# pymc-devs/pymc

Measured on AMD Instinct MI355X. Metric: effective samples/sec (and leapfrog steps/sec), 10k-param hierarchical logistic regression, one NUTS chain per GPU, higher is better.
Workload: dtype f64

## Files before the change

### pymc_amd/csrc/engine.hip

```cpp
#include <hip/hip_runtime.h>

#include <algorithm>
#include <atomic>
#include <chrono>
#include <cmath>
#include <cstdio>
#include <cstdlib>
#include <cstring>
#include <mutex>
#include <thread>
#include <utility>
#include <ctime>
#include <string>
#include <vector>

#include "kernels.h"
#include "small_kernel.h"
#include "mixture_kernel.h"
#include "nuts_mi355.h"
#include "pcg64_stream.h"
#include "advi.h"

static thread_local std::string g_err;

// ... 1135 lines not shown
      const auto& uses = cs.lin_uses[l][k];
      if (uses.size() > LIN_MAXUSE) { g_err = "a linear predictor column is read by too many factors (LIN_MAXUSE)"; return false; }
      C.n_use = (int32_t)uses.size();
      for (size_t u = 0; u < uses.size(); ++u) { C.adj_off[u] = uses[u].adj_off; C.use_size[u] = uses[u].size; }
      const int64_t last = (int64_t)L.off[k] + (int64_t)(L.P - 1) * L.stride[k];
      if (L.off[k] < 0 || L.stride[k] < 0 || (L.stride[k] == 0 && L.P > 1)) { g_err = "linear predictor: bad coefficient offset / stride"; return false; }
      double* dst_base = nullptr; int64_t cbase = 0;
      if (L.var[k] >= 0) {
        if (L.var[k] >= md.n_vars) { g_err = "linear predictor refers to a missing variable"; return false; }
        const VarDev& v = cs.vars[L.var[k]];
        if (last >= v.size) { g_err = "linear predictor: coefficients beyond the end of their variable"; return false; }
        C.transform = v.transform; C.lower = v.lower; C.upper = v.upper;
        cbase = v.offset; dst_base = md.lin_gdense + v.offset;
      } else {
        const int fi = -(L.var[k] + 1);
        int t = -1;
        for (int u = 0; u < md.n_derived; ++u) if (md.derived_f[u] == fi) t = u;
        if (t < 0) { g_err = "linear predictor: coefficients must be a variable or a NUTS_D_DERIVED factor"; return false; }
        const int64_t sz = cs.fac[fi].size;
        if (last >= sz) { g_err = "linear predictor: coefficients beyond the end of their derived vector"; return false; }
        C.transform = -1; C.lower = 0.0; C.upper = 0.0;
        cbase = md.derived_off[t]; dst_base = const_cast<double*>(md.pool) + md.derived_off[t] + sz;
      }
      for (int p = 0; p < L.P; ++p) {
        const int64_t e = (int64_t)L.off[k] + (int64_t)p * L.stride[k];
        coef[(size_t)k * L.P + p] = (int32_t)(cbase + e);
        if (C.n_use > 0) srcs.push_back(Src{(int64_t)reinterpret_cast<intptr_t>(dst_base + e), LinSrc{l, k, p, 0}, dst_base + e});
      }
    }
    D.coef = m->keep(dev_upload(coef.data(), coef.size()));
    m->alg_bytes += 16 * L.N * (int64_t)L.P;
  }
  std::stable_sort(srcs.begin(), srcs.end(), [](const Src& a, const Src& b) { return a.key < b.key; });
  std::vector<LinTarget> targets;
  std::vector<LinSrc> flat;
  for (size_t i = 0; i < srcs.size(); ++i) {
    if (i == 0 || srcs[i].key != srcs[i - 1].key) targets.push_back(LinTarget{srcs[i].dst, (int32_t)flat.size(), 0});
    targets.back().n_src++;
    flat.push_back(srcs[i].src);
  }
  md.n_lins = s->n_lins; md.n_lin_targets = (int32_t)targets.size();
  md.lins = m->keep(dev_upload(m->lins_host.data(), m->lins_host.size()));
  md.lin_targets = m->keep(dev_upload(targets.data(), targets.size()));
  md.lin_srcs = m->keep(dev_upload(flat.data(), flat.size()));
  return true;
}

static bool build_rows_group(nuts_model* m, const nuts_model_spec* s, const std::vector<int64_t>& gptr, const std::vector<int32_t>& tile0,
                             int64_t maxT, int W, int gpw) {
  RowsDev& lg = m->md.lg;
  const int n = m->md.n, D = lg.D, SPAN = WAVE * m->rows_rpl;
  const int64_t n_tiles = tile0[lg.G];
  lg.ga = 1; lg.ga_w = gpw ? GB_W : W;
  lg.ga_gpw = gpw;
  lg.ga_bsz = gpw ? gpw : (lg.G + 31) / 32;
  lg.ga_flags = env_int("NUTS_GA_FLAGS", 0);
  lg.ga_T_uni = 0; lg.ga_ng_uni = 0;
  {
    bool uni = lg.G > 0;
    for (int g = 1; g < lg.G; ++g) uni = uni && (gptr[g + 1] - gptr[g] == gptr[1] - gptr[0]);
    if (uni && maxT > 0) { lg.ga_T_uni = (int32_t)maxT; lg.ga_ng_uni = gptr[1] - gptr[0]; }
  }
  lg.ga_nblk = (lg.G + lg.ga_bsz - 1) / lg.ga_bsz;
  lg.ga_auxel = n - lg.G * D;
  lg.ga_naux = m->ga_struct_ok == 2 ? (lg.ga_auxel + WAVE * lg.ga_w - 1) / (WAVE * lg.ga_w) : 0;
  lg.ga_nrec = lg.ga_nblk + lg.ga_naux;
  bool ones0 = D == 8 && env_int("NUTS_GA_ONES0", 1) != 0 && lg.N > 0;
  for (int64_t i = 0; ones0 && i < lg.N; ++i) ones0 = s->rows_X[i * D] == 1.0;
  const int DX = ones0 ? D - 1 : D;
  lg.ga_dx = DX;
  const int64_t TS = (int64_t)DX * SPAN, GA_SKEW = env_int("NUTS_GA_SKEW", DX == 7 || DX == 5 ? 1120 : 1056);
  if (GA_SKEW % DX != 0) return refuse("NUTS_GA_SKEW must be a multiple of the stored column count");
  std::vector<int64_t> coff((size_t)lg.G * W, 0);
  int64_t pos = 0, max_ct = 0;
  for (int g = 0; g < lg.G; ++g) {
    const int64_t T = tile0[g + 1] - tile0[g];
    for (int w = 0; w < W; ++w) {
      const int64_t ct = (int64_t)(w + 1) * T / W - (int64_t)w * T / W;
      coff[(size_t)g * W + w] = pos;
      pos += ct * TS + GA_SKEW;
      max_ct = std::max(max_ct, ct);
    }
  }
  lg.ga_cstride_uni = 0;
  if (lg.ga_T_uni > 0 && lg.ga_T_uni % W == 0) {
    lg.ga_cstride_uni = (lg.ga_T_uni / W) * TS + GA_SKEW;
  } else lg.ga_T_uni = 0;
  lg.Npad = n_tiles * SPAN; lg.n_spans = n_tiles;
  std::vector<double> xt((size_t)(pos + TS), 0.0);
  std::vector<int8_t> yy((size_t)(pos / DX + 2 * SPAN), 0);
  for (int g = 0; g < lg.G; ++g) {
    const int64_t T = tile0[g + 1] - tile0[g];
    for (int64_t i = gptr[g]; i < gptr[g + 1]; ++i) {
      const int64_t r = i - gptr[g], t = r / SPAN, rr = r % SPAN;
      int w = (int)(((t + 1) * W - 1) / std::max<int64_t>(T, 1));
      while (w > 0 && (int64_t)w * T / W > t) --w;
      while (w + 1 < W && (int64_t)(w + 1) * T / W <= t) ++w;
      const int64_t base = coff[(size_t)g * W + w] + (t - (int64_t)w * T / W) * TS;
      for (int d = D - DX; d < D; ++d) xt[(size_t)(base + (int64_t)(d - (D - DX)) * SPAN + rr)] = s->rows_X[i * D + d];
      yy[(size_t)(base / DX + rr)] = s->rows_y[i];
    }
  }
  lg.Xt = m->keep(dev_upload(xt.data(), xt.size()));
  lg.y = m->keep(dev_upload(yy.data(), yy.size()));
  m->rows_xt_len = (int64_t)xt.size(); m->rows_y_len = (int64_t)yy.size();
  lg.ga_coff = m->keep(dev_upload(coff.data(), coff.size()));
  lg.ga_tile0 = m->keep(dev_upload(tile0.data(), tile0.size()));
  lg.ga_part = m->keep(dev_alloc<double>((size_t)lg.G * PART_STRIDE));
  const size_t bpart_len = gpw ? 2 * (size_t)PART_STRIDE * ((lg.ga_nrec + WAVE - 1) / WAVE * WAVE) : 2 * (size_t)lg.ga_nrec * PART_STRIDE;
  lg.ga_bpart = m->keep(dev_alloc<double>(bpart_len));
  lg.ga_ticket = m->keep(dev_alloc<unsigned>(lg.ga_nblk));
  if (lg.ga_part) hipMemset(lg.ga_part, 0, (size_t)lg.G * PART_STRIDE * sizeof(double));
  if (lg.ga_bpart) hipMemset(lg.ga_bpart, 0, bpart_len * sizeof(double));
  if (lg.ga_ticket) hipMemset(lg.ga_ticket, 0, lg.ga_nblk * sizeof(unsigned));
  m->rows_grid = gpw ? lg.ga_nblk : lg.G;
  return true;
}

static bool build_rows_spans(nuts_model* m, const nuts_model_spec* s, int cus) {
  RowsDev& lg = m->md.lg;
  const int D = lg.D, SPAN = WAVE * m->rows_rpl;
  const int32_t* gid = s->rows_gid;
  int wpc = env_int("NUTS_ROWS_WAVES_PER_CU", 0);
  if (wpc <= 0) {
    const int64_t spans = (s->rows_N + (int64_t)WAVE * m->rows_rpl - 1) / ((int64_t)WAVE * m->rows_rpl);
    wpc = spans >= (int64_t)cus * 32 * 4 ? 32 : 16;
  }
  {
    std::vector<double> xt((size_t)D * lg.Npad, 0.0);
    for (int64_t i = 0; i < lg.N; ++i) {
      const int64_t sp = i / SPAN, r = i % SPAN;
      for (int d = 0; d < D; ++d) xt[((size_t)sp * D + d) * SPAN + r] = s->rows_X[i * D + d];
    }
    lg.Xt = m->keep(dev_upload(xt.data(), xt.size()));
  }
  std::vector<int8_t> yy(lg.Npad, 0);
  for (int64_t i = 0; i < lg.N; ++i) yy[i] = s->rows_y[i];
  lg.y = m->keep(dev_upload(yy.data(), yy.size()));
  const int waves_per_block = ROWS_BLOCK / WAVE;
  int64_t want_waves = std::min<int64_t>((int64_t)cus * wpc, lg.n_spans);
  const int nb_main = (int)((want_waves + waves_per_block - 1) / waves_per_block);
  lg.n_waves = nb_main * waves_per_block;
  std::vector<int32_t> span_gid(lg.n_spans), mixed_g0, mixed_seg_base, mixed_seg_gid;
  std::vector<int64_t> mixed_span;
  for (int64_t sp = 0; sp < lg.n_spans; ++sp) {
    const int64_t r0 = sp * SPAN, r1 = r0 + SPAN;
    if (r1 <= lg.N && gid[r0] == gid[r1 - 1]) { span_gid[sp] = gid[r0]; continue; }
    span_gid[sp] = -1;
    mixed_span.push_back(sp);
    mixed_g0.push_back(gid[r0]);
    mixed_seg_base.push_back((int32_t)mixed_seg_gid.size());
    int prev = -1;
    for (int64_t r = r0; r < std::min<int64_t>(r1, lg.N); ++r)
      if (gid[r] != prev) { prev = gid[r]; mixed_seg_gid.push_back(prev); }
  }
  lg.n_mixed = (int32_t)mixed_span.size();
  lg.n_mixed_seg = (int32_t)mixed_seg_gid.size();
  std::vector<int32_t> run_ptr(lg.n_waves + 1, 0), seg_gid;
  std::vector<int4> runs;
  for (int w = 0; w < lg.n_waves; ++w) {
    const int64_t s0 = (int64_t)w * lg.n_spans / lg.n_waves, s1 = (int64_t)(w + 1) * lg.n_spans / lg.n_waves;
    run_ptr[w] = (int32_t)runs.size();
    for (int64_t sp = s0; sp < s1; ++sp) {
      if (span_gid[sp] < 0) continue;
      if (!runs.empty() && (int)runs.size() > run_ptr[w] && runs.back().z == span_gid[sp] && runs.back().x + runs.back().y == sp) {
        runs.back().y++;
// ... 354 lines not shown
  if (hipGetDeviceCount(&ndev) != hipSuccess || ndev == 0) {
    g_err = "no HIP device visible: libnuts_mi355 requires an MI355X (gfx950); there is no CPU fallback";
    return nullptr;
  }
  auto* m = new nuts_model();
  if (!model_build(m, s)) { nuts_model_destroy(m); return nullptr; }
  return m;
}

extern "C" int nuts_model_set_data(nuts_model* m, int32_t data_id, const double* values, int64_t n) {
  if (!m || !values) { g_err = "null argument"; return NUTS_E_ARG; }
  if (data_id < 0 || data_id >= (int)m->data_refs.size()) { g_err = "nuts_model_set_data: no such data vector"; return NUTS_E_ARG; }
  const nuts_data_ref& r = m->data_refs[data_id];
  if (n != r.size) { g_err = "nuts_model_set_data: the length of a data vector cannot change"; return NUTS_E_ARG; }
  HIPCHK(hipStreamSynchronize(m->stream));
  HIPCHK(hipMemcpy(const_cast<double*>(m->md.pool) + r.offset, values, (size_t)n * sizeof(double), hipMemcpyHostToDevice));
  m->data_epoch++;
  return NUTS_OK;
}

extern "C" int nuts_model_set_data_many(nuts_model* m, int32_t count, const int32_t* data_ids, const double* values, const int64_t* lens) {
  if (!m || count < 0 || (count > 0 && (!data_ids || !values || !lens))) { g_err = "null argument"; return NUTS_E_ARG; }
  int64_t total = 0;
  for (int i = 0; i < count; ++i) {
    if (data_ids[i] < 0 || data_ids[i] >= (int)m->data_refs.size()) { g_err = "nuts_model_set_data_many: no such data vector"; return NUTS_E_ARG; }
    if (lens[i] != m->data_refs[data_ids[i]].size) { g_err = "nuts_model_set_data_many: the length of a data vector cannot change"; return NUTS_E_ARG; }
    total += lens[i];
  }
  if (total == 0) return NUTS_OK;
  if (m->set_pin_len < total) {
    if (m->set_ev) HIPCHK(hipEventSynchronize(m->set_ev));
    if (m->set_pin) hipHostFree(m->set_pin);
    m->set_pin = nullptr; m->set_pin_len = 0;
    HIPCHK(hipHostMalloc((void**)&m->set_pin, (size_t)total * sizeof(double), hipHostMallocDefault));
    m->set_pin_len = total;
  }
  if (!m->set_ev) HIPCHK(hipEventCreateWithFlags(&m->set_ev, hipEventDisableTiming));
  else HIPCHK(hipEventSynchronize(m->set_ev));
  std::memcpy(m->set_pin, values, (size_t)total * sizeof(double));
  int64_t at = 0;
  for (int i = 0; i < count;) {
    const int64_t off0 = m->data_refs[data_ids[i]].offset;
    int64_t run = lens[i];
    int j = i + 1;
    while (j < count && m->data_refs[data_ids[j]].offset == off0 + run) { run += lens[j]; ++j; }
    if (run > 0)
      HIPCHK(hipMemcpyAsync(const_cast<double*>(m->md.pool) + off0, m->set_pin + at, (size_t)run * sizeof(double), hipMemcpyHostToDevice, m->stream));
    at += run;
    i = j;
  }
  HIPCHK(hipEventRecord(m->set_ev, m->stream));
  m->data_epoch++;
  return NUTS_OK;
}

static void group_remove_model(struct nuts_group* g, nuts_model* m);
extern "C" void nuts_model_destroy(nuts_model* m) {
  if (!m) return;
  if (m->stream) hipStreamSynchronize(m->stream);
  if (m->set_ev) hipEventDestroy(m->set_ev);
  if (m->set_pin) hipHostFree(m->set_pin);
  if (m->group) group_remove_model(m->group, m);
  for (void* p : m->owned) if (p) hipFree(p);
  for (auto e : m->ev) hipEventDestroy(e);
  if (m->host_pin) hipHostFree(m->host_pin);
  if (m->own_stream) hipStreamDestroy(m->own_stream);
  delete m;
}

extern "C" int nuts_model_debug_ticks(nuts_model* m, int64_t* out) {
  if (!m || !out) return NUTS_E_ARG;
  HIPCHK(hipStreamSynchronize(m->stream));
  HIPCHK(hipMemcpy(out, m->md.ticks, 64 * sizeof(long long), hipMemcpyDeviceToHost));
  return NUTS_OK;
}

extern "C" int32_t nuts_model_ndim(const nuts_model* m) { return m ? m->md.n : -1; }
extern "C" int nuts_model_get_scalar(const nuts_model* m, const char* name, double* out) {
  if (!m || !name || !out) return NUTS_E_ARG;
  const std::string k(name);
  if (k == "rows_group_aligned") *out = m->md.lg.ga;
  else if (k == "rows_group_block") *out = m->md.lg.ga_gpw;
  else if (k == "rows_aux_workgroups") *out = m->md.lg.ga ? m->md.lg.ga_naux : 0;
  else if (k == "mixture_workgroups") *out = m->md.has_mix ? m->md.mix.nwg : 0;
  else if (k == "glm_workgroups") *out = m->md.has_glm ? m->md.glm.nwg : 0;
  else if (k == "glm_row_stride") *out = m->md.has_glm ? m->md.glm.xstride : 0;
  else if (k == "glm_layout_width") *out = m->md.has_glm ? m->md.glm.Ppad : 0;
  else if (k == "mvn_row_aligned") *out = m->md.has_mvn ? m->md.mv.aligned : 0;
  else if (k == "rows_waves") *out = m->md.lg.ga ? m->md.lg.ga_w : m->md.lg.n_waves;
  else if (k == "lean") *out = m->md.lean_ok;
  else if (k == "chain_group_kind") {
    const RowsDev& lg = m->md.lg;
    const bool is_mvn = m->md.has_mvn && (m->md.mv.aligned == 4 || m->md.mv.aligned == 8 || m->md.mv.aligned == 16);
    const bool is_rows = m->md.has_logit && !m->md.has_mvn && lg.ga && lg.ga_naux == 0 && lg.D == 8 && m->ga_struct_ok == 1;
    *out = is_mvn ? 1.0 : (is_rows ? (lg.ga_gpw > 0 ? 3.0 : 2.0) : 0.0);
  }
  else if (k == "chain_group_wide_ok") *out = (m->md.has_mvn && m->md.mv.aligned > 0 && m->md.mv.k % 16 == 0) ? 1.0 : 0.0;
  else if (k == "chain_group_wide_rows") *out = 8.0;
  else if (k == "single_workgroup_ok") *out = (m->md.n <= SMALL_MAX_N && m->ept == 1 && !m->md.has_logit && !m->md.has_mvn && !m->md.has_mix && !m->md.has_glm && m->md.n_lins == 0 && m->factor_elems <= SMALL_MAX_ELEMS) ? 1.0 : 0.0;
  else { g_err = "unknown model scalar " + k; return NUTS_E_ARG; }
  return NUTS_OK;
}
extern "C" int64_t nuts_model_algorithmic_bytes(const nuts_model* m) { return m ? m->alg_bytes : 0; }

extern "C" int nuts_model_logp_grad(nuts_model* m, const double* q, double* logp, double* grad) {
  if (!m || !q || !logp) { g_err = "null argument"; return NUTS_E_ARG; }
  const int n = m->md.n;
  std::memcpy(m->host_pin, q, n * sizeof(double));
  HIPCHK(hipMemcpyAsync(m->q_dev, m->host_pin, n * sizeof(double), hipMemcpyHostToDevice, m->stream));
  m->md.fdead_mode = 1;
  model_enqueue_plain(m, m->q_dev, m->g_dev, m->lp_dev);
  m->md.fdead_mode = 0;
  HIPCHK(hipMemcpyAsync(m->host_pin + n, m->g_dev, n * sizeof(double), hipMemcpyDeviceToHost, m->stream));
  HIPCHK(hipMemcpyAsync(m->host_pin + 2 * n, m->lp_dev, sizeof(double), hipMemcpyDeviceToHost, m->stream));
  HIPCHK(hipStreamSynchronize(m->stream));
  HIPCHK(hipGetLastError());
  *logp = m->host_pin[2 * n];
  if (m->md.n_factors > 0 && !std::isfinite(*logp)) {
    std::vector<int32_t> fd(m->md.n_factors);
    HIPCHK(hipMemcpy(fd.data(), m->md.fdead, fd.size() * sizeof(int32_t), hipMemcpyDeviceToHost));
    bool any = false;
    for (int32_t v : fd) any = any || v != 0;
    if (any) {
      if (grad) {
        m->md.fdead_mode = 2;
        model_enqueue_plain(m, m->q_dev, m->g_dev, m->lp_dev);
        m->md.fdead_mode = 0;
        HIPCHK(hipMemcpyAsync(m->host_pin + n, m->g_dev, n * sizeof(double), hipMemcpyDeviceToHost, m->stream));
      }
      HIPCHK(hipMemsetAsync(m->md.fdead, 0, fd.size() * sizeof(int32_t), m->stream));
      HIPCHK(hipStreamSynchronize(m->stream));
      HIPCHK(hipGetLastError());
    }
  }
  if (grad) std::memcpy(grad, m->host_pin + n, n * sizeof(double));
  return NUTS_OK;
}

static void profile_enable(nuts_model* m, bool on, int sample_every, size_t max_pairs) {
  m->profile = on;
  m->sample_every = std::max(1, sample_every);
  m->ev_used = 0;
  m->dom_launches = 0;
  m->dom_units = 0;
  m->run_open = 0; m->runs_seen = 0;
  while (on && m->ev.size() < 2 * max_pairs) {
    hipEvent_t e;
    hipEventCreate(&e);
    m->ev.push_back(e);
  }
  m->ev_units.assign(m->ev.size() / 2 + 1, 1);
}
static double profile_sum_ms(nuts_model* m, int64_t* pairs) {
  std::vector<float> ms(m->ev_used / 2, 0.f);
  std::vector<double> run_avg;
  for (size_t i = 0; i + 1 < m->ev_used; i += 2) {
    if (hipEventElapsedTime(&ms[i / 2], m->ev[i], m->ev[i + 1]) != hipSuccess) ms[i / 2] = -1.f;
    else if (m->ev_units[i / 2] > 1) run_avg.push_back(ms[i / 2] / m->ev_units[i / 2]);
  }
  double med = 0.0;
  if (!run_avg.empty()) { std::sort(run_avg.begin(), run_avg.end()); med = run_avg[run_avg.size() / 2]; }
  double tot = 0.0;
  int64_t units = 0, kept = 0;
  for (size_t p = 0; p < ms.size(); ++p) {
    if (ms[p] < 0.f) continue;
    const int u = m->ev_units[p];
// ... 2070 lines not shown
```

### pymc_amd/csrc/model_dev.h

```cpp
#pragma once
#include "device_math.h"
#include "nuts_mi355.h"

#define MAX_BTERMS 8
#define MAX_DERIVED 4
#define MAX_FACTOR_BT 6
#define MAX_DEFERRED 256
#define LOGIT_MAXD 8
#define SEG_MAIN_MAX 10

struct VarDev {
  int32_t offset, size, transform, deferred;
  double lower, upper;
  int32_t normal_prior;
  int32_t def_base;
  double np_mu, np_inv_var, np_lognorm;
};

struct Contrib {
  int32_t f;
  int16_t arg, slot;
  int32_t owner;
  int32_t fast;
  int32_t dist, pad;
  double konst;
  double p[4];
};

#define MAX_GSLOTS 64
struct GSlot { int32_t var, did; int64_t adj_off; };
struct GSweepFactor { int32_t f, slot0, n_slots, elem0; int32_t orphan, pad; };
#define GADJ_LONG 512
#define GADJ_CHUNK 4096
struct GLong { int64_t adj_off; int32_t lst_off, len; int32_t nchunk, pad; };

struct FactorBT {
  int32_t n, pad;
  struct { int16_t arg, slot; int32_t bterm; } e[MAX_FACTOR_BT];
};

struct RowsDev {
  int64_t N, Npad;
  int32_t D, G;
  const double* Xt;
  const int8_t* y;
  const int64_t* gptr;
  int32_t off_mu, off_sigma, off_z, sigma_tr;
  int32_t var_mu, var_sigma, var_z, pad;
  int32_t def_mu, def_sigma;
  int32_t segK, seg_pad;
  int64_t n_spans;
  int32_t n_waves, n_seg;
  const int32_t* run_ptr;
  const int4* runs;
  const int32_t* gseg_ptr;
  double* seg_part;
  int32_t n_mixed, n_mixed_seg;
  const int64_t* mixed_span;
  const int32_t* mixed_g0;
  const int32_t* mixed_seg_base;
  const int32_t* gmix_ptr;
  double* mixed_part;
  double* wave_lp;
  int32_t ga, ga_w;
  int32_t ga_dx, ga_gpw;
  int32_t ga_nblk, ga_bsz;
  int32_t ga_T_uni, ga_flags;
  int64_t ga_ng_uni;
  const int32_t* ga_tile0;
  const int64_t* ga_coff;
  int64_t ga_cstride_uni;
  unsigned* ga_ticket;
  double* ga_part;
  double* ga_bpart;
  int32_t ga_naux, ga_nrec, ga_auxel, ga_pad2;
  double z_np_mu, z_np_inv_var, z_np_lognorm;
  double mu_c[3];
  double sg_c[2];
};

struct MvnDev {
  int32_t k, off;
  const double* mu;
  const double* prec;
  double konst;
  double* rowq;
  double* gdense;
  const double* winv; const double* winv_t;
  double* wy;
  int32_t aligned, al_nwg;
  double* al_part;
};

#define MIX_MAXK 16
struct MixDev {
  int64_t N;
  int32_t K, off_mu, off_sigma, off_w;
  int32_t tr_sigma, nwg;
  int32_t w_simplex, pad_;
  double alpha[MIX_MAXK], w_konst;
  const double* y;
  const double* assign;
  double sigma_c[MIX_MAXK], logw_c[MIX_MAXK];
  double* part;
  double* gdense;
  double* lp;
};

struct GlmDev {
  int64_t N;
  int32_t P, Ppad;
  int32_t xstride, xpad_;
  int32_t family, lpr, ch;
  int32_t off_beta, off_icpt, off_sigma, tr_sigma, nwg;
  const double* beta_buf; double* beta_seed;
  double sigma_c;
  double konst;
  const double* X;
  const double* Xt;
  const double* y;
  double* part;
  double* gdense;
  double* lp;
};

#define SW_LEAF 6
#define SWL_DATA 0
#define SWL_GATHER 1
// ... 909 lines not shown
```

### pymc_amd/csrc/rows_ga_kernel.h

```cpp
#pragma once
#include "rows_kernel.h"

__device__ __forceinline__ void ga_def_local(const RowsDev& R, bool is_mu, double qn, double& gx, double& dxdq, double& dj, double& lp) {
  if (is_mu) {
    const double r = qn - R.mu_c[0];
    const double z = r * R.mu_c[1];
    lp = -0.5 * z * z - R.mu_c[2] + (-0.91893853320467274178);
    gx = -z * R.mu_c[1]; dxdq = 1.0; dj = 0.0;
  } else {
    double x, lj;
    if (R.sigma_tr == NUTS_TR_LOG) { x = exp(qn); dxdq = x; lj = qn; dj = 1.0; }
    else { x = qn; dxdq = 1.0; lj = 0.0; dj = 0.0; }
    const double z = x * R.sg_c[0];
    double lpf = -0.5 * z * z - R.sg_c[1] + (-0.22579135264472743236);
    double g = -z * R.sg_c[0];
    if (!(x >= 0)) { lpf = -INFINITY; g = 0.0; }
    gx = g; lp = lj + lpf;
  }
}

template <int D, int RPL>
__device__ __forceinline__ void ga_load(const RowsDev& R, int64_t xoff, int lane, double (&x)[D][RPL], uint32_t& ybits) {
  constexpr int SPAN = WAVE * RPL;
  const double* tile = R.Xt + xoff + lane * RPL;
  const int8_t* yp = R.y + xoff / D + lane * RPL;
  if (RPL == 2) ybits = *reinterpret_cast<const uint16_t*>(yp);
  else ybits = *reinterpret_cast<const uint32_t*>(yp);
#pragma unroll
  for (int d = 0; d < D; ++d) {
#pragma unroll
    for (int k = 0; k < RPL; k += 2) {
      const double2 a = *reinterpret_cast<const double2*>(tile + d * SPAN + k);
      x[d][k] = a.x; x[d][k + 1] = a.y;
    }
  }
}

typedef double ga_v2d __attribute__((ext_vector_type(2)));
struct GaTileRegs { ga_v2d c[8]; uint32_t y; };

__device__ __forceinline__ void ga_issue8(const double* base , const int8_t* ybase,
                                          uint32_t voff16, uint32_t voff2, GaTileRegs& t) {
  const double* base2 = base + 512;
  asm volatile(
      "s_nop 4\n\t"
      "global_load_dwordx4 %0, %9, %10\n\t"
      "global_load_dwordx4 %1, %9, %10 offset:1024\n\t"
      "global_load_dwordx4 %2, %9, %10 offset:2048\n\t"
      "global_load_dwordx4 %3, %9, %10 offset:3072\n\t"
      "global_load_dwordx4 %4, %9, %11\n\t"
      "global_load_dwordx4 %5, %9, %11 offset:1024\n\t"
      "global_load_dwordx4 %6, %9, %11 offset:2048\n\t"
      "global_load_dwordx4 %7, %9, %11 offset:3072\n\t"
      "global_load_ushort %8, %12, %13"
      : "=&v"(t.c[0]), "=&v"(t.c[1]), "=&v"(t.c[2]), "=&v"(t.c[3]), "=&v"(t.c[4]), "=&v"(t.c[5]), "=&v"(t.c[6]), "=&v"(t.c[7]), "=&v"(t.y)
      : "v"(voff16), "s"(base), "s"(base2), "v"(voff2), "s"(ybase)
      : "memory");
}

template <int N>
__device__ __forceinline__ void ga_wait8(GaTileRegs& t) {
  asm volatile("s_waitcnt vmcnt(%9)"
               : "+v"(t.c[0]), "+v"(t.c[1]), "+v"(t.c[2]), "+v"(t.c[3]), "+v"(t.c[4]), "+v"(t.c[5]), "+v"(t.c[6]), "+v"(t.c[7]), "+v"(t.y)
               : "i"(N));
}

struct GaTileRegs7 { ga_v2d c[7]; uint32_t y; };

__device__ __forceinline__ void ga_issue8(const double* base, const int8_t* ybase, uint32_t voff16, uint32_t voff2, GaTileRegs7& t) {
  const double* base2 = base + 512;
  asm volatile(
      "s_nop 4\n\t"
      "global_load_dwordx4 %0, %8, %9\n\t"
      "global_load_dwordx4 %1, %8, %9 offset:1024\n\t"
      "global_load_dwordx4 %2, %8, %9 offset:2048\n\t"
      "global_load_dwordx4 %3, %8, %9 offset:3072\n\t"
      "global_load_dwordx4 %4, %8, %10\n\t"
      "global_load_dwordx4 %5, %8, %10 offset:1024\n\t"
      "global_load_dwordx4 %6, %8, %10 offset:2048\n\t"
      "global_load_ushort %7, %11, %12"
      : "=&v"(t.c[0]), "=&v"(t.c[1]), "=&v"(t.c[2]), "=&v"(t.c[3]), "=&v"(t.c[4]), "=&v"(t.c[5]), "=&v"(t.c[6]), "=&v"(t.y)
      : "v"(voff16), "s"(base), "s"(base2), "v"(voff2), "s"(ybase)
      : "memory");
}

template <int N>
__device__ __forceinline__ void ga_wait8(GaTileRegs7& t) {
  asm volatile("s_waitcnt vmcnt(%8)"
               : "+v"(t.c[0]), "+v"(t.c[1]), "+v"(t.c[2]), "+v"(t.c[3]), "+v"(t.c[4]), "+v"(t.c[5]), "+v"(t.c[6]), "+v"(t.y)
               : "i"(N));
}

__device__ __forceinline__ void ga_unpack(const GaTileRegs& t, double (&xx)[8][2]) {
#pragma unroll
  for (int dd = 0; dd < 8; ++dd) { xx[dd][0] = t.c[dd].x; xx[dd][1] = t.c[dd].y; }
}
__device__ __forceinline__ void ga_unpack(const GaTileRegs7& t, double (&xx)[8][2]) {
  xx[0][0] = 1.0; xx[0][1] = 1.0;
#pragma unroll
  for (int dd = 1; dd < 8; ++dd) { xx[dd][0] = t.c[dd - 1].x; xx[dd][1] = t.c[dd - 1].y; }
}
template <int DX> struct GaTileSel { typedef GaTileRegs type; };
template <> struct GaTileSel<7> { typedef GaTileRegs7 type; };

template <int D, int RPL, bool ILV = false>
__device__ __forceinline__ void ga_tile(const double (&x)[D][RPL], uint32_t yb, const double (&beta)[D], int nvalid, int lane,
                                        double (&acc)[D], double& lp) {
  if constexpr (ILV && RPL == 2) {
    double eta[2] = {0.0, 0.0}, yk[2], l[2], rr[2];
#pragma unroll
    for (int d = 0; d < D; ++d) { eta[0] = fma(x[d][0], beta[d], eta[0]); eta[1] = fma(x[d][1], beta[d], eta[1]); }
    yk[0] = (double)(yb & 0xffu); yk[1] = (double)((yb >> 8) & 0xffu);
    logit_row2(eta, yk, l, rr);
#pragma unroll
    for (int k = 0; k < 2; ++k) {
      const bool in = lane * 2 + k < nvalid;
      lp += in ? l[k] : 0.0;
      rr[k] = in ? rr[k] : 0.0;
    }
#pragma unroll
    for (int d = 0; d < D; ++d) { acc[d] = fma(rr[0], x[d][0], acc[d]); acc[d] = fma(rr[1], x[d][1], acc[d]); }
    return;
  }
#pragma unroll
  for (int k = 0; k < RPL; ++k) {
    double eta = 0.0;
#pragma unroll
    for (int d = 0; d < D; ++d) eta = fma(x[d][k], beta[d], eta);
    double l, rr;
    logit_row(eta, (double)((yb >> (8 * k)) & 0xffu), l, rr);
    const bool in = lane * RPL + k < nvalid;
    lp += in ? l : 0.0;
    rr = in ? rr : 0.0;
#pragma unroll
    for (int d = 0; d < D; ++d) acc[d] = fma(rr, x[d][k], acc[d]);
    if constexpr (!ILV) __builtin_amdgcn_sched_barrier(0);
  }
}

#define GA_MAXW 4
#define GA_MAXCHUNK 8
#define GA_F_NOTAIL 1

struct GaArgs;
template <int D>
__device__ __forceinline__ void ga_tail(const GaArgs& T, int g, double (&s_acc)[4][2][D + 1], double (&s_red)[NDOT],
                                        double (&s_cp)[8][PART_STRIDE], int (&s_info)[4], double (&s_keep)[5][WAVE]);

struct GaArgs {
  ModelDev md; ArenaDev A; EvalIO io;
  int j, rev, fold, par, d, max_depth;
  double Emax;
  HostStatus* st;
  EvalIO cio;
  int cj, cd, cseq, cpad;
};
#define GA_FOLD_CTL 1
#define GA_FOLD_SRC 2
#include "rows_aux.h"

template <int D>
__device__ __forceinline__ void ga_hyper(const ModelDev& md, const QView& qv, int fold, int par, int lane, double& hval0, double& hph0) {
  const RowsDev& R = md.lg;
  if (fold & GA_FOLD_SRC) {
    const LeanSrc prev = lean_src(md, par ^ 1);
    rows_hyper_fold_elem<D>(R, prev.part, prev.stride, prev.nblk, prev.def_loc, qv, lane, hval0, hph0);
  } else {
    const int e = lane % (2 * D);
    const int i = e < D ? R.off_mu + e : R.off_sigma + (e - D);
    if (qv.composed) { hph0 = qv.p_half(i); hval0 = fma(qv.eps, qv.var[i] * hph0, qv.q[i]); }
    else { hph0 = 0.0; hval0 = qv.q[i]; }
  }
}

template <int D, int RPL, int DX = D>
__global__ __launch_bounds__(64 * GA_MAXW, 4) void k_rows_ga(GaArgs a) {
  constexpr int SPAN = WAVE * RPL;
  static_assert(DX == D || (D == 8 && DX == 7), "only the intercept column of an 8-column model is elided");
  typedef typename GaTileSel<DX>::type Tile;
  constexpr int LOADS = DX + 1;
  const ModelDev& md = a.md;
  const ArenaDev& A = a.A;
  const EvalIO& io = a.io;
  const int j = a.j, rev = a.rev, fold = a.fold, par = a.par, d = a.d, max_depth = a.max_depth;
  const double Emax = a.Emax;
  HostStatus* const st = a.st;
  const RowsDev& R = md.lg;
  int b = (int)blockIdx.x;
  if (fold & GA_FOLD_CTL) {
    if (b == 0) { control_lean(md, A, a.cio, a.cj, a.cd, Emax, max_depth, st, a.cseq, lean_src(md, par ^ 1)); return; }
    --b;
  }
  const int g = b;
  const int tid = threadIdx.x, lane = tid & (WAVE - 1), w = __builtin_amdgcn_readfirstlane(tid >> 6), W = (int)blockDim.x >> 6;
  Leaf lf; QView qv;
  const int aborted = load_aborted(io, A);
  resolve_leaf(io, A, j, lf, qv);
  const bool leaf = io.mode != MODE_PLAIN;
  __shared__ double s_acc[GA_MAXW][2][D + 1];
  __shared__ double s_red[NDOT];
  __shared__ double s_cp[GA_MAXCHUNK][PART_STRIDE];
  __shared__ int s_info[4];
  __shared__ double s_keep[5][WAVE];
  __shared__ __attribute__((aligned(16))) char s_args[(sizeof(GaArgs) + 15) / 16 * 16];
  __shared__ __attribute__((aligned(16))) char s_auxprog[GA_AUX_PROG_LDS];
  if (b >= R.G) {
    static_assert(GA_AUX_SCRATCH_DOUBLES(GA_MAXW) <= GA_MAXCHUNK * PART_STRIDE, "auxiliary scratch does not fit the chunk buffer");
    double hv, hp;
    ga_hyper<D>(md, qv, fold, par, lane, hv, hp);
    const int aux_id = b - R.G;
    ga_aux<4>((const GaArgs*)__builtin_amdgcn_kernarg_segment_ptr(), aux_id, hv, hp, &s_cp[0][0], GA_MAXW, s_auxprog,
                R.ga_bpart + ((int64_t)par * R.ga_nrec + R.ga_nblk + aux_id) * PART_STRIDE, 1);
    return;
  }

  int T; int64_t ng, cbase;
  if (R.ga_T_uni > 0) { T = R.ga_T_uni; ng = R.ga_ng_uni; cbase = (int64_t)(g * W + w) * R.ga_cstride_uni; }
  else {
    T = __builtin_amdgcn_readfirstlane(R.ga_tile0[g + 1] - R.ga_tile0[g]);
    ng = __builtin_amdgcn_readfirstlane((int)(R.gptr[g + 1] - R.gptr[g]));
    const int64_t cb = R.ga_coff[g * W + w];
    cbase = ((int64_t)__builtin_amdgcn_readfirstlane((int)(cb >> 32)) << 32) | (uint32_t)__builtin_amdgcn_readfirstlane((int)(cb & 0xffffffffll));
  }
  const int c0 = (int)((int64_t)w * T / W), c2 = (int)((int64_t)(w + 1) * T / W);
  const int n = c2 - c0;
  const int nA = (n + 1) / 2;
  const int nsw = rev ? n - nA : nA;
  constexpr int64_t TS = (int64_t)DX * SPAN;
  auto local_at = [&](int i) { return rev ? (i < nsw ? nA + i : i - nsw) : i; };
  auto tile_at = [&](int i) { return cbase + (int64_t)local_at(i) * TS; };
  const int l_last = (c2 == T) ? n - 1 : -1;
  const int n_last = (int)(ng - (int64_t)(T - 1) * SPAN);
  double xa[D][RPL], xb[D][RPL];
  uint32_t ya = 0, yb = 0;
  Tile ta, tb;
  if constexpr (D == 8 && RPL == 2) {
    const uint32_t voff16 = (uint32_t)lane * 16u, voff2 = (uint32_t)lane * 2u;
    const int64_t o0 = tile_at(0), o1 = tile_at(min(1, max(n - 1, 0)));
    ga_issue8(R.Xt + o0, R.y + o0 / DX, voff16, voff2, ta);
    ga_issue8(R.Xt + o1, R.y + o1 / DX, voff16, voff2, tb);
  } else {
    ga_load<D, RPL>(R, tile_at(0), lane, xa, ya);
  }
  if (lane == 0) {
#pragma unroll
    for (int dd = 0; dd <= D; ++dd) { s_acc[w][0][dd] = 0.0; s_acc[w][1][dd] = 0.0; }
  }
  {
    const uint4* ka = (const uint4*)__builtin_amdgcn_kernarg_segment_ptr();
    for (int t = tid; t < (int)((sizeof(GaArgs) + 15) / 16); t += (int)blockDim.x) reinterpret_cast<uint4*>(s_args)[t] = ka[t];
  }
  __syncthreads();

  double hval0, hph0;
  ga_hyper<D>(md, qv, fold, par, lane, hval0, hph0);
  const int dl = lane % D;
  const int iz = R.off_z + g * D + dl;
  double beta[D];
  {
    double zq, zph;
    if (qv.composed) { zph = fma(qv.half, qv.g[iz], qv.p[iz]); zq = fma(qv.eps, qv.var[iz] * zph, qv.q[iz]); }
    else { zph = 0.0; zq = qv.q[iz]; }
    const double m_lane = __shfl(hval0, dl);
    const double sraw = __shfl(hval0, D + dl);
    const double s_lane = R.sigma_tr == NUTS_TR_LOG ? exp(sraw) : sraw;
    const double bl = fma(s_lane, zq, m_lane);
#pragma unroll
    for (int dd = 0; dd < D; ++dd) beta[dd] = readlane_d(bl, dd);
    if (w == 0) { s_keep[0][lane] = hval0; s_keep[1][lane] = hph0; s_keep[2][lane] = zq; s_keep[3][lane] = zph; s_keep[4][lane] = s_lane; }
  }
  if (aborted) return;

  {
    double acc[D], lp = 0.0;
#pragma unroll
    for (int dd = 0; dd < D; ++dd) acc[dd] = 0.0;
    int half = rev ? 1 : 0;
    auto flush = [&]() {
#pragma unroll
      for (int dd = 0; dd < D; ++dd) {
        const double sum = wave_sum(acc[dd]);
        if (lane == 0) s_acc[w][half][dd] = sum;
        acc[dd] = 0.0;
      }
      const double sum = wave_sum(lp);
      if (lane == 0) s_acc[w][half][D] = sum;
      lp = 0.0;
      half ^= 1;
    };
#define GA_STAGE(X, Y, I)                                                                   \
    {                                                                                        \
      if ((I) == nsw) flush();                                                               \
      ga_tile<D, RPL>(X, Y, beta, local_at(I) == l_last ? n_last : SPAN, lane, acc, lp);     \
    }
    const int nm1 = n - 1;
    if constexpr (D == 8 && RPL == 2) {
      const uint32_t voff16 = (uint32_t)lane * 16u, voff2 = (uint32_t)lane * 2u;
      auto issue = [&](int i, Tile& t) {
        const int64_t off = tile_at(min(i, nm1));
        ga_issue8(R.Xt + off, R.y + off / DX, voff16, voff2, t);
      };
#define GA_ASTAGE(T, I)                                                                      \
      {                                                                                      \
        ga_wait8<LOADS>(T);                                                                  \
        if ((I) == nsw) flush();                                                             \
        double xx[8][2];                                                                     \
        ga_unpack(T, xx);                                                                    \
        ga_tile<8, 2>(xx, T.y, beta, local_at(I) == l_last ? n_last : SPAN, lane, acc, lp); \
      }
      for (int i = 0; i < n; i += 2) {
        GA_ASTAGE(ta, i)
        if (i + 1 >= n) break;
        issue(i + 2, ta);
        GA_ASTAGE(tb, i + 1)
        issue(i + 3, tb);
      }
      ga_wait8<0>(ta); ga_wait8<0>(tb);
#undef GA_ASTAGE
    } else {
      for (int i = 0; i < n; i += 2) {
        ga_load<D, RPL>(R, tile_at(min(i + 1, nm1)), lane, xb, yb);
        GA_STAGE(xa, ya, i)
        if (i + 1 >= n) break;
        ga_load<D, RPL>(R, tile_at(min(i + 2, nm1)), lane, xa, ya);
        GA_STAGE(xb, yb, i + 1)
      }
    }
#undef GA_STAGE
    if (n > 0) flush();
  }

  ga_tail<D>(*reinterpret_cast<const GaArgs*>(s_args), g, s_acc, s_red, s_cp, s_info, s_keep);
}

template <int D>
__device__ __forceinline__ void ga_tail(const GaArgs& T, int g, double (&s_acc)[GA_MAXW][2][D + 1], double (&s_red)[NDOT],
                                        double (&s_cp)[GA_MAXCHUNK][PART_STRIDE], int (&s_info)[4], double (&s_keep)[5][WAVE]) {
  const ModelDev& md = T.md;
  const ArenaDev& A = T.A;
  const EvalIO& io = T.io;
  const RowsDev& R = md.lg;
  const int j = T.j, par = T.par, d = T.d;
  const int tid = threadIdx.x, lane = tid & (WAVE - 1), w = tid >> 6, W = (int)blockDim.x >> 6;
  Leaf lf; QView qv;
  resolve_leaf(io, A, j, lf, qv);
  const bool leaf = io.mode != MODE_PLAIN;
  const bool tree = io.mode == MODE_TREE;
  const int dl = lane % D;
  const int iz = R.off_z + g * D + dl;
  MergePrefetch mpf;
  if (w == 0 && tree && !(R.ga_flags & GA_F_NOTAIL)) merge_prefetch(A, lf, j, iz, mpf);
  __syncthreads();
  if (R.ga_flags & GA_F_NOTAIL) return;

  if (w == 0) {
    const double hval = s_keep[0][lane], hph = s_keep[1][lane], zq = s_keep[2][lane], zph = s_keep[3][lane], s_lane = s_keep[4][lane];
    double db = 0.0, lpg = 0.0;
    for (int ww = 0; ww < W; ++ww) { db += s_acc[ww][0][dl] + s_acc[ww][1][dl]; lpg += s_acc[ww][0][D] + s_acc[ww][1][D]; }
    const bool zact = lane < D;
    int idx[1] = {iz};
    bool act[1] = {zact};
    double grad[1] = {0.0}, ph[1] = {zph};
    {
      const double r = zq - R.z_np_mu;
      const double gx = -r * R.z_np_inv_var;
      const double lpz = -0.5 * r * r * R.z_np_inv_var - R.z_np_lognorm;
      grad[0] = gx + s_lane * db;
      lpg += wave_sum(zact ? lpz : 0.0);
      if (zact) {
        if (leaf) { A.G[lf.d_o + iz] = grad[0]; A.Q[lf.d_o + iz] = zq; }
        else io.grad[iz] = grad[0];
      }
    }
    if (g == 0 && R.ga_naux == 0) {
      const int e = lane;
      const bool hact = e < 2 * D, is_mu = e < D;
      double gx, dxdq, dj, lpd;
      ga_def_local(R, is_mu, hval, gx, dxdq, dj, lpd);
      lpg += wave_sum(hact ? lpd : 0.0);
      if (hact) {
        const int dd = is_mu ? e : e - D;
        const int slot = (is_mu ? R.def_mu : R.def_sigma) + dd;
        double2* loc = reinterpret_cast<double2*>(md.def_loc + (int64_t)par * 4 * MAX_DEFERRED) + 2 * slot;
        loc[0] = make_double2(gx, dxdq);
        loc[1] = make_double2(dj, hph);
        if (leaf) A.Q[lf.d_o + (is_mu ? R.off_mu : R.off_sigma) + dd] = hval;
      }
    }
    int m = 0; bool last = false;
    if (leaf) leaf_post<1>(A, lf, j, d, tree, idx, act, grad, ph, s_red, 1, m, last, tree ? &mpf : nullptr);
    __builtin_amdgcn_fence(__ATOMIC_RELEASE, "wavefront");
    __builtin_amdgcn_wave_barrier();

    double* rec = R.ga_part + (int64_t)g * PART_STRIDE;
    if (lane == 0) st_agent(rec + PART_LP, lpg);
    if (zact) { st_agent(rec + PART_DMU + lane, db); st_agent(rec + PART_DSG + lane, db * zq); }
    if (leaf) {
      for (int k = lane; k < NDOT; k += WAVE)
        if (dot_needed(k, m, last)) st_agent(rec + PART_DOT + k, s_red[k]);
    }
    asm volatile("s_waitcnt vmcnt(0)" ::: "memory");

    const int blk = g / R.ga_bsz;
    const int cnt = min(R.G, (blk + 1) * R.ga_bsz) - blk * R.ga_bsz;
    unsigned old = 0;
    if (lane == 0) old = __hip_atomic_fetch_add(&R.ga_ticket[blk], 1u, __ATOMIC_RELAXED, __HIP_MEMORY_SCOPE_AGENT);
    old = (unsigned)__builtin_amdgcn_readfirstlane((int)old);
    const int is_last = (int)old + 1 == cnt;
    if (is_last && lane == 0) __hip_atomic_store(&R.ga_ticket[blk], 0u, __ATOMIC_RELAXED, __HIP_MEMORY_SCOPE_AGENT);
    if (lane == 0) { s_info[0] = is_last; s_info[1] = m; s_info[2] = last ? 1 : 0; }
  }
  __syncthreads();
  if (!s_info[0]) return;

  {
    const int m = s_info[1];
    const bool last = s_info[2] != 0;
    const int blk = g / R.ga_bsz, g0 = blk * R.ga_bsz;
    const int cnt = min(R.G, g0 + R.ga_bsz) - g0;
    const int nch = (cnt + 7) / 8;
    const int nn = 1 + 2 * D + (leaf ? 1 + 6 * m + (last ? 6 : 0) : 0);
    auto need_slot = [&](int q) {
      if (q < 1) return PART_LP;
      if (q < 1 + D) return PART_DMU + (q - 1);
      if (q < 1 + 2 * D) return PART_DSG + (q - 1 - D);
      if (q < 1 + 2 * D + 1 + 6 * m) return PART_DOT + (q - 1 - 2 * D);
      return PART_DOT + DOT_TOP + (q - 1 - 2 * D - 1 - 6 * m);
    };
    const int NT = (int)blockDim.x;
    for (int p = tid; p < nn * nch; p += NT) {
      const int c = p / nn, k = need_slot(p - c * nn);
      const int gg0 = c * 8, gcnt = min(8, cnt - gg0);
      const double* src = R.ga_part + (int64_t)(g0 + gg0) * PART_STRIDE + k;
      double v[8];
#pragma unroll
      for (int u = 0; u < 8; ++u) v[u] = ld_agent(src + (int64_t)min(u, gcnt - 1) * PART_STRIDE);
      double sum = 0.0;
#pragma unroll
      for (int u = 0; u < 8; ++u) sum += (u < gcnt) ? v[u] : 0.0;
      s_cp[c][k] = sum;
    }
    __syncthreads();
    double* bp = R.ga_bpart + ((int64_t)par * R.ga_nrec + blk) * PART_STRIDE;
    for (int q = tid; q < nn; q += NT) {
      const int k = need_slot(q);
      double sum = 0.0;
      for (int c = 0; c < nch; ++c) sum += s_cp[c][k];
      bp[k] = sum;
    }
  }
}
```

Before: 17980.

## Compute group-aligned chunk offsets in closed form and hoist tile loads before leaf setup

When groups are uniform, each wave's chunk base and its y offset are now computed from precomputed strides held in RowsDev, replacing loads from the chunk offset table and a 64-bit divide. The first tile loads are issued before the abort-flag read and leaf resolution, and the abort flag is fetched with a non-blocking load that is waited on later, so that global memory latency overlaps with setup. Padding lanes of the last tile now reuse lane 0's address instead of reading past the valid rows. Optional s_memtime instrumentation is added behind a compile flag, and the host checks the closed-form geometry against the table, refusing the model if they disagree.

```diff
diff --git a/pymc_amd/csrc/engine.hip b/pymc_amd/csrc/engine.hip
--- a/pymc_amd/csrc/engine.hip
+++ b/pymc_amd/csrc/engine.hip
@@ -1241,6 +1241,23 @@
       max_ct = std::max(max_ct, ct);
     }
   }
+  const int edges = env_int("NUTS_GA_EDGES", 1);
+  static_assert(sizeof(lg.ga_e_c0) / sizeof(lg.ga_e_c0[0]) == GA_MAXW + 1, "RowsDev.ga_e_c0 holds GA_MAXW + 1 first tiles");
+  lg.ga_e_on = edges != 0; lg.ga_e_pad0 = edges == 1 || edges == 3;
+  const bool edges_geo = edges == 1 || edges == 2;
+  lg.ga_e_uni = 0; lg.ga_e_gstride = 0; lg.ga_e_gstride_y = 0; lg.ga_e_skew = 0; lg.ga_e_skew_y = 0; lg.ga_e_nlast = 0; lg.ga_e_T = 0;
+  for (int w = 0; w <= GA_MAXW; ++w) lg.ga_e_c0[w] = 0;
+  if (edges_geo && !gpw && lg.ga_T_uni > 0 && W <= GA_MAXW && GA_SKEW > 0 && GA_SKEW < ((int64_t)1 << 31)) {
+    const int64_t T = lg.ga_T_uni;
+    lg.ga_e_uni = 1; lg.ga_e_T = (int32_t)T;
+    lg.ga_e_gstride = T * TS + W * GA_SKEW; lg.ga_e_gstride_y = lg.ga_e_gstride / DX;
+    lg.ga_e_skew = (int32_t)GA_SKEW; lg.ga_e_skew_y = (int32_t)(GA_SKEW / DX);
+    lg.ga_e_nlast = (int32_t)(lg.ga_ng_uni - (T - 1) * SPAN);
+    for (int w = 0; w <= W; ++w) lg.ga_e_c0[w] = (int32_t)((int64_t)w * T / W);
+    for (int g = 0; g < lg.G; ++g)
+      for (int w = 0; w < W; ++w)
+        if (coff[(size_t)g * W + w] != g * lg.ga_e_gstride + lg.ga_e_c0[w] * TS + w * GA_SKEW) return refuse("group-aligned rows: closed-form chunk geometry does not match the chunk table");
+  }
   lg.ga_cstride_uni = 0;
   if (lg.ga_T_uni > 0 && lg.ga_T_uni % W == 0) {
     lg.ga_cstride_uni = (lg.ga_T_uni / W) * TS + GA_SKEW;
@@ -1761,6 +1778,7 @@
   if (k == "rows_group_aligned") *out = m->md.lg.ga;
   else if (k == "rows_group_block") *out = m->md.lg.ga_gpw;
   else if (k == "rows_aux_workgroups") *out = m->md.lg.ga ? m->md.lg.ga_naux : 0;
+  else if (k == "rows_ga_edges") *out = (m->md.lg.ga && m->md.lg.ga_e_on) ? 1 + m->md.lg.ga_e_uni : 0;
   else if (k == "mixture_workgroups") *out = m->md.has_mix ? m->md.mix.nwg : 0;
   else if (k == "glm_workgroups") *out = m->md.has_glm ? m->md.glm.nwg : 0;
   else if (k == "glm_row_stride") *out = m->md.has_glm ? m->md.glm.xstride : 0;
diff --git a/pymc_amd/csrc/model_dev.h b/pymc_amd/csrc/model_dev.h
--- a/pymc_amd/csrc/model_dev.h
+++ b/pymc_amd/csrc/model_dev.h
@@ -44,6 +44,10 @@
   int32_t D, G;
   const double* Xt;
   const int8_t* y;
+  int64_t ga_e_gstride, ga_e_gstride_y;
+  int32_t ga_e_c0[5];
+  int32_t ga_e_skew, ga_e_skew_y, ga_e_nlast, ga_e_T;
+  int32_t ga_e_on, ga_e_uni, ga_e_pad0;
   const int64_t* gptr;
   int32_t off_mu, off_sigma, off_z, sigma_tr;
   int32_t var_mu, var_sigma, var_z, pad;
diff --git a/pymc_amd/csrc/rows_ga_kernel.h b/pymc_amd/csrc/rows_ga_kernel.h
--- a/pymc_amd/csrc/rows_ga_kernel.h
+++ b/pymc_amd/csrc/rows_ga_kernel.h
@@ -20,10 +20,10 @@
 }
 
 template <int D, int RPL>
-__device__ __forceinline__ void ga_load(const RowsDev& R, int64_t xoff, int lane, double (&x)[D][RPL], uint32_t& ybits) {
+__device__ __forceinline__ void ga_load(const RowsDev& R, int64_t xoff, int64_t yoff, int lane, double (&x)[D][RPL], uint32_t& ybits) {
   constexpr int SPAN = WAVE * RPL;
   const double* tile = R.Xt + xoff + lane * RPL;
-  const int8_t* yp = R.y + xoff / D + lane * RPL;
+  const int8_t* yp = R.y + yoff + lane * RPL;
   if (RPL == 2) ybits = *reinterpret_cast<const uint16_t*>(yp);
   else ybits = *reinterpret_cast<const uint32_t*>(yp);
 #pragma unroll
@@ -65,6 +65,11 @@
                : "i"(N));
 }
 
+__device__ __forceinline__ void ga_issue_flag(const int* flag , uint32_t& v) {
+  asm volatile("global_load_dword %0, %1, %2 sc1" : "=&v"(v) : "v"(0u), "s"(flag) : "memory");
+}
+__device__ __forceinline__ void ga_wait_flag(uint32_t& v) { asm volatile("s_waitcnt vmcnt(0)" : "+v"(v)); }
+
 struct GaTileRegs7 { ga_v2d c[7]; uint32_t y; };
 
 __device__ __forceinline__ void ga_issue8(const double* base, const int8_t* ybase, uint32_t voff16, uint32_t voff2, GaTileRegs7& t) {
@@ -141,6 +146,23 @@
 #define GA_MAXW 4
 #define GA_MAXCHUNK 8
 #define GA_F_NOTAIL 1
+
+#ifdef NUTS_KTIMING
+__device__ __forceinline__ long long* ga_tk_buf() { __shared__ long long s_tk[8]; return s_tk; }
+__device__ __forceinline__ void ga_tk(bool on, int slot) {
+  if (on) {
+    unsigned long long t;
+    asm volatile("s_memtime %0\n\ts_waitcnt lgkmcnt(0)" : "=s"(t) :: "memory");
+    if (slot == 0) { for (int k = 1; k < 8; ++k) ga_tk_buf()[k] = 0; }
+    ga_tk_buf()[slot] = (long long)t;
+  }
+}
+#define GA_TK(on, slot) ga_tk(on, slot)
+#define GA_TK_OUT(md, on) do { if (on) { for (int k_ = 0; k_ < 8; ++k_) (md).ticks[k_] = ga_tk_buf()[k_]; } } while (0)
+#else
+#define GA_TK(on, slot) do { } while (0)
+#define GA_TK_OUT(md, on) do { } while (0)
+#endif
 
 struct GaArgs;
 template <int D>
@@ -194,9 +216,9 @@
   const int g = b;
   const int tid = threadIdx.x, lane = tid & (WAVE - 1), w = __builtin_amdgcn_readfirstlane(tid >> 6), W = (int)blockDim.x >> 6;
   Leaf lf; QView qv;
-  const int aborted = load_aborted(io, A);
-  resolve_leaf(io, A, j, lf, qv);
   const bool leaf = io.mode != MODE_PLAIN;
+  const bool tk = b == R.G / 2 && tid == 0 && (md.tick_j < 0 || j == md.tick_j);
+  GA_TK(tk, 0);
   __shared__ double s_acc[GA_MAXW][2][D + 1];
   __shared__ double s_red[NDOT];
   __shared__ double s_cp[GA_MAXCHUNK][PART_STRIDE];
@@ -207,6 +229,7 @@
   if (b >= R.G) {
     static_assert(GA_AUX_SCRATCH_DOUBLES(GA_MAXW) <= GA_MAXCHUNK * PART_STRIDE, "auxiliary scratch does not fit the chunk buffer");
     double hv, hp;
+    resolve_leaf(io, A, j, lf, qv);
     ga_hyper<D>(md, qv, fold, par, lane, hv, hp);
     const int aux_id = b - R.G;
     ga_aux<4>((const GaArgs*)__builtin_amdgcn_kernarg_segment_ptr(), aux_id, hv, hp, &s_cp[0][0], GA_MAXW, s_auxprog,
@@ -214,34 +237,55 @@
     return;
   }
 
-  int T; int64_t ng, cbase;
-  if (R.ga_T_uni > 0) { T = R.ga_T_uni; ng = R.ga_ng_uni; cbase = (int64_t)(g * W + w) * R.ga_cstride_uni; }
-  else {
-    T = __builtin_amdgcn_readfirstlane(R.ga_tile0[g + 1] - R.ga_tile0[g]);
-    ng = __builtin_amdgcn_readfirstlane((int)(R.gptr[g + 1] - R.gptr[g]));
-    const int64_t cb = R.ga_coff[g * W + w];
-    cbase = ((int64_t)__builtin_amdgcn_readfirstlane((int)(cb >> 32)) << 32) | (uint32_t)__builtin_amdgcn_readfirstlane((int)(cb & 0xffffffffll));
-  }
-  const int c0 = (int)((int64_t)w * T / W), c2 = (int)((int64_t)(w + 1) * T / W);
+  constexpr int64_t TS = (int64_t)DX * SPAN;
+  int T, c0, c2, n_last; int64_t cbase, cby;
+  if (R.ga_e_uni) {
+    static_assert(GA_MAXW == 4, "the select chains below and RowsDev.ga_e_c0[GA_MAXW + 1] are written for four waves");
+    const int k0 = R.ga_e_c0[0], k1 = R.ga_e_c0[1], k2 = R.ga_e_c0[2], k3 = R.ga_e_c0[3], k4 = R.ga_e_c0[4];
+    c0 = w == 0 ? k0 : (w == 1 ? k1 : (w == 2 ? k2 : k3));
+    c2 = w == 0 ? k1 : (w == 1 ? k2 : (w == 2 ? k3 : k4));
+    T = R.ga_e_T; n_last = R.ga_e_nlast;
+    cbase = (int64_t)g * R.ga_e_gstride + (int64_t)c0 * TS + (int64_t)w * R.ga_e_skew;
+    cby = (int64_t)g * R.ga_e_gstride_y + (int64_t)c0 * SPAN + (int64_t)w * R.ga_e_skew_y;
+  } else {
+    int64_t ng;
+    if (R.ga_T_uni > 0) { T = R.ga_T_uni; ng = R.ga_ng_uni; cbase = (int64_t)(g * W + w) * R.ga_cstride_uni; }
+    else {
+      T = __builtin_amdgcn_readfirstlane(R.ga_tile0[g + 1] - R.ga_tile0[g]);
+      ng = __builtin_amdgcn_readfirstlane((int)(R.gptr[g + 1] - R.gptr[g]));
+      const int64_t cb = R.ga_coff[g * W + w];
+      cbase = ((int64_t)__builtin_amdgcn_readfirstlane((int)(cb >> 32)) << 32) | (uint32_t)__builtin_amdgcn_readfirstlane((int)(cb & 0xffffffffll));
+    }
+    c0 = (int)((int64_t)w * T / W); c2 = (int)((int64_t)(w + 1) * T / W);
+    n_last = (int)(ng - (int64_t)(T - 1) * SPAN);
+    cby = cbase / DX;
+  }
   const int n = c2 - c0;
   const int nA = (n + 1) / 2;
   const int nsw = rev ? n - nA : nA;
-  constexpr int64_t TS = (int64_t)DX * SPAN;
   auto local_at = [&](int i) { return rev ? (i < nsw ? nA + i : i - nsw) : i; };
   auto tile_at = [&](int i) { return cbase + (int64_t)local_at(i) * TS; };
+  auto y_at = [&](int i) { return cby + (int64_t)local_at(i) * SPAN; };
   const int l_last = (c2 == T) ? n - 1 : -1;
-  const int n_last = (int)(ng - (int64_t)(T - 1) * SPAN);
+  const int n_fetch = R.ga_e_pad0 ? n_last : SPAN;
   double xa[D][RPL], xb[D][RPL];
   uint32_t ya = 0, yb = 0;
   Tile ta, tb;
+  auto issue_at = [&](int i, Tile& t) {
+    const bool pad = local_at(i) == l_last && lane * RPL >= n_fetch;
+    ga_issue8(R.Xt + tile_at(i), R.y + y_at(i), pad ? 0u : (uint32_t)lane * 16u, pad ? 0u : (uint32_t)lane * 2u, t);
+  };
   if constexpr (D == 8 && RPL == 2) {
-    const uint32_t voff16 = (uint32_t)lane * 16u, voff2 = (uint32_t)lane * 2u;
-    const int64_t o0 = tile_at(0), o1 = tile_at(min(1, max(n - 1, 0)));
-    ga_issue8(R.Xt + o0, R.y + o0 / DX, voff16, voff2, ta);
-    ga_issue8(R.Xt + o1, R.y + o1 / DX, voff16, voff2, tb);
+    issue_at(0, ta);
+    GA_TK(tk, 1);
+    issue_at(min(1, max(n - 1, 0)), tb);
   } else {
-    ga_load<D, RPL>(R, tile_at(0), lane, xa, ya);
-  }
+    ga_load<D, RPL>(R, tile_at(0), y_at(0), lane, xa, ya);
+  }
+  const bool in_tree = io.mode == MODE_TREE;
+  uint32_t aborted;
+  ga_issue_flag(in_tree ? &A.ctl->aborted : (const int*)__builtin_amdgcn_kernarg_segment_ptr(), aborted);
+  resolve_leaf(io, A, j, lf, qv);
   if (lane == 0) {
 #pragma unroll
     for (int dd = 0; dd <= D; ++dd) { s_acc[w][0][dd] = 0.0; s_acc[w][1][dd] = 0.0; }
@@ -269,7 +313,9 @@
     for (int dd = 0; dd < D; ++dd) beta[dd] = readlane_d(bl, dd);
     if (w == 0) { s_keep[0][lane] = hval0; s_keep[1][lane] = hph0; s_keep[2][lane] = zq; s_keep[3][lane] = zph; s_keep[4][lane] = s_lane; }
   }
-  if (aborted) return;
+  GA_TK(tk, 3);
+  ga_wait_flag(aborted);
+  if (in_tree && __builtin_amdgcn_readfirstlane((int)aborted)) return;
 
   {
     double acc[D], lp = 0.0;
@@ -295,14 +341,11 @@
     }
     const int nm1 = n - 1;
     if constexpr (D == 8 && RPL == 2) {
-      const uint32_t voff16 = (uint32_t)lane * 16u, voff2 = (uint32_t)lane * 2u;
-      auto issue = [&](int i, Tile& t) {
-        const int64_t off = tile_at(min(i, nm1));
-        ga_issue8(R.Xt + off, R.y + off / DX, voff16, voff2, t);
-      };
+      auto issue = [&](int i, Tile& t) { issue_at(min(i, nm1), t); };
 #define GA_ASTAGE(T, I)                                                                      \
       {                                                                                      \
         ga_wait8<LOADS>(T);                                                                  \
+        GA_TK(tk && (I) == 0, 2);                                                            \
         if ((I) == nsw) flush();                                                             \
         double xx[8][2];                                                                     \
         ga_unpack(T, xx);                                                                    \
@@ -319,16 +362,17 @@
 #undef GA_ASTAGE
     } else {
       for (int i = 0; i < n; i += 2) {
-        ga_load<D, RPL>(R, tile_at(min(i + 1, nm1)), lane, xb, yb);
+        ga_load<D, RPL>(R, tile_at(min(i + 1, nm1)), y_at(min(i + 1, nm1)), lane, xb, yb);
         GA_STAGE(xa, ya, i)
         if (i + 1 >= n) break;
-        ga_load<D, RPL>(R, tile_at(min(i + 2, nm1)), lane, xa, ya);
+        ga_load<D, RPL>(R, tile_at(min(i + 2, nm1)), y_at(min(i + 2, nm1)), lane, xa, ya);
         GA_STAGE(xb, yb, i + 1)
       }
     }
 #undef GA_STAGE
     if (n > 0) flush();
   }
+  GA_TK(tk, 4);
 
   ga_tail<D>(*reinterpret_cast<const GaArgs*>(s_args), g, s_acc, s_red, s_cp, s_info, s_keep);
 }
@@ -348,6 +392,7 @@
   const bool tree = io.mode == MODE_TREE;
   const int dl = lane % D;
   const int iz = R.off_z + g * D + dl;
+  const bool tk = g == R.G / 2 && tid == 0 && (md.tick_j < 0 || j == md.tick_j);
   MergePrefetch mpf;
   if (w == 0 && tree && !(R.ga_flags & GA_F_NOTAIL)) merge_prefetch(A, lf, j, iz, mpf);
   __syncthreads();
@@ -400,6 +445,7 @@
         if (dot_needed(k, m, last)) st_agent(rec + PART_DOT + k, s_red[k]);
     }
     asm volatile("s_waitcnt vmcnt(0)" ::: "memory");
+    GA_TK(tk, 5);
 
     const int blk = g / R.ga_bsz;
     const int cnt = min(R.G, (blk + 1) * R.ga_bsz) - blk * R.ga_bsz;
@@ -411,7 +457,8 @@
     if (lane == 0) { s_info[0] = is_last; s_info[1] = m; s_info[2] = last ? 1 : 0; }
   }
   __syncthreads();
-  if (!s_info[0]) return;
+  GA_TK(tk, 6);
+  if (!s_info[0]) { GA_TK_OUT(md, tk); return; }
 
   {
     const int m = s_info[1];
@@ -449,4 +496,6 @@
       bp[k] = sum;
     }
   }
-}
+  GA_TK(tk, 7);
+  GA_TK_OUT(md, tk);
+}
```

New measurement: 18890 (median of 6 runs). 1.05x the previous value.
